# voxel-tracer/cuda-raytracing-optimized

Measured on AMD Instinct MI355X. Metric: Msamples/s (pixels x spp / s), random-spheres 1200x800x100spp, higher is better.
Workload: dtype f32; 1 GPU; random-spheres (488 spheres, LCG seed 0) 1200x800 100spp maxDepth 50, gradient sky, reference RNG stream, fp parity; spp=100, max_depth=50, spheres=488, partition=single GPU, fp_mode=parity, rng=reference, kernel_variant=0

## Files before the change

### cuda-raytracing-optimized_amd/csrc/rt_kernels_spheres.hip

```cpp
#include "rt_device.h"
#include "rt_params.h"

#include <float.h>
#include <cstdio>
#include <cstdlib>
#include <algorithm>
#include <utility>

using namespace rtd;

#if defined(RT_MODE_PARITY)
#define RT_LAUNCH_NAME rt_launch_spheres_parity
#elif defined(RT_MODE_FAST)
#define RT_LAUNCH_NAME rt_launch_spheres_fast
#else
#error "define RT_MODE_PARITY or RT_MODE_FAST"
#endif

namespace {

#ifndef RT_BOX_CUT
#define RT_BOX_CUT 12
#endif
constexpr int kWavesPerWg = 16;
// ... 95 lines not shown
    }
    for (int k = threadIdx.x; k < 3 * P.n_groups + rt_cell_f4(P.n_groups); k += (int)blockDim.x) s_grp[k] = P.groups[k];
    for (int k = threadIdx.x; k < P.n; k += (int)blockDim.x) s_sof[k] = P.slot_of[k];
    float* s_fb = reinterpret_cast<float*>(s_sof + ((P.n + 3) & ~3));
    *after = s_fb;
    unsigned char* scratch = reinterpret_cast<unsigned char*>(s_fb + (WITH_FB ? kThreads * 3 : 0));
    __syncthreads();
    return { s_sph, s_grp, s_mat, s_typ, s_org, s_sof, s_rad, scratch };
}

struct Lane {
    uint32_t rng;
    f3 col;
    f3 org, dir, atten;
    int bounce;
    bool inside;
    int s;
    int i, j;
    uint32_t pixelId;
};

struct SampleParams { rt_camera cam; int32_t nx, ny, rng_mode; };
template <bool COUNTER = true, typename PP>
__device__ __forceinline__ void start_sample(const PP& P, Lane& L) {
    if (COUNTER && P.rng_mode == RT_RNG_COUNTER) L.rng = sample_seed(L.pixelId, (uint32_t)L.s);
    const float u = ((float)L.i + rnd(L.rng)) / (float)P.nx;
    const float v = ((float)L.j + rnd(L.rng)) / (float)P.ny;
    f3 d;
    get_ray(P.cam, u, v, L.rng, L.org, d);
    L.dir = unit(d);
    L.atten = F3(1.0f, 1.0f, 1.0f);
    L.bounce = 0;
    L.inside = false;
}

__device__ __forceinline__ void init_pixel(const RtSphereParams& P, Lane& L, int i, int j, int first_sample = 0) {
    L.i = i; L.j = j;
    L.pixelId = (uint32_t)(j * P.nx + i);
    L.rng = pixel_seed(L.pixelId);
    L.col = F3(0, 0, 0);
    L.s = first_sample;
}

__device__ __forceinline__ void start_pixel(const RtSphereParams& P, Lane& L, int i, int j, int first_sample = 0) {
    init_pixel(P, L, i, j, first_sample);
    start_sample(P, L);
}

__device__ __forceinline__ void scan_group_broadcast(const RtSphereParams& P, const SceneLds& S, int g, f3 org, f3 dn, float a, Hit& h) {
    const int base = g << kSphereGroupShift;
    const float4* sp = S.sph + sidx(base);
    uint32_t mask = 0;
#pragma unroll
    for (int kk = 0; kk < kSphereGroup; kk++) {
        const float4 sph = sp[kk];
        const float ocx = org.x - sph.x;
        const float ocy = org.y - sph.y;
        const float ocz = org.z - sph.z;
        const float b = ocx * dn.x + ocy * dn.y + ocz * dn.z;
        const float c = (ocx * ocx + ocy * ocy + ocz * ocz) - sph.w;
        const float nd = a * c - b * b;
        mask = __builtin_amdgcn_alignbit(mask, __float_as_uint(nd), 31);
    }
    mask <<= (32 - kSphereGroup);
    while (mask) {
        const int lz = __clz((int)mask);
// ... 511 lines not shown
        if (reach) {
            const int at = np + (int)__builtin_amdgcn_mbcnt_hi((uint32_t)(rm >> 32), __builtin_amdgcn_mbcnt_lo((uint32_t)rm, 0u));
            w_pair[at] = (unsigned short)((r << 12) | g);
        }
        np += (int)__popcll(rm);
    }
    __builtin_amdgcn_fence(__ATOMIC_ACQ_REL, "wavefront");
    __builtin_amdgcn_wave_barrier();
    lap(12);
    for (int base = 0; base < (np << kSphereGroupShift); base += 64) {
        const int w = base + lane;
        if (w < (np << kSphereGroupShift)) {
            const unsigned pr = w_pair[w >> kSphereGroupShift];
            const int r = (int)(pr >> 12), g = (int)(pr & 0xFFFu);
            const float4 ro = w_ray[r], rd = w_ray[64 + r];
            sparse_test_slot(P, S, (g << kSphereGroupShift) + (w & (kSphereGroup - 1)), F3(ro.x, ro.y, ro.z), F3(rd.x, rd.y, rd.z), ro.w, &w_best[r]);
        }
    }
    __builtin_amdgcn_fence(__ATOMIC_ACQ_REL, "wavefront");
    __builtin_amdgcn_wave_barrier();
    Hit out = { FLT_MAX, -1, 0x7fffffff };
    if (mine) {
        const unsigned long long key = w_best[my_r];
        if (key != ~0ull) {
            out.closest = __uint_as_float((uint32_t)(key >> 32));
            out.orig = (int)(uint32_t)key;
            out.sid = S.slot_of[out.orig];
        }
    }
    lap(13);
    return out;
}

__device__ __forceinline__ Hit scan_single(const RtSphereParams& P, const SceneLds& S, int q, f3 org, f3 dn, float a) {
    const int lane = threadIdx.x & 63;
    auto bc = [&](float v) { return __int_as_float(__builtin_amdgcn_readlane(__float_as_int(v), q)); };
    const f3 O = F3(bc(org.x), bc(org.y), bc(org.z)), D = F3(bc(dn.x), bc(dn.y), bc(dn.z));
    const float A = bc(a);
    const float Ak = A - 3.814697265625e-6f;
    const int rounds = P.n_padded >> 6;
    uint32_t mask = 0;
#pragma unroll 4
    for (int r = 0; r < rounds; r++) {
        const float4 sph = S.sph[sidx((r << 6) + lane)];
        const f3 oc = O - F3(sph.x, sph.y, sph.z);
        const float b = __builtin_fmaf(oc.z, D.z, __builtin_fmaf(oc.y, D.y, oc.x * D.x));
        const float c = __builtin_fmaf(oc.z, oc.z, __builtin_fmaf(oc.y, oc.y, __builtin_fmaf(oc.x, oc.x, -sph.w)));
        const float v = __builtin_fmaf(Ak, c, -__builtin_fmaf(b, b, 7.62939453125e-6f * sph.w));
        mask |= (__float_as_uint(v) >> 31) << r;
    }
    Hit h = { FLT_MAX, -1, 0x7fffffff };
    while (mask) {
        const int r = __builtin_ctz(mask);
        mask &= mask - 1u;
        const int k = (r << 6) + lane;
        const float t = sphere_hit_exact(S.sph[sidx(k)], O, D, A, P.t_min, FLT_MAX);
        const int o = S.orig[k];
        if (o != 0x7fffffff && t < FLT_MAX) accept(h, t, k, o);
    }
    unsigned long long found = __ballot(h.closest < FLT_MAX);
    uint32_t st = __float_as_uint(FLT_MAX);
    int sk = -1, so = 0x7fffffff;
    while (found) {
        const int bq = __builtin_ctzll(found);
        found &= found - 1;
        const uint32_t tb = (uint32_t)__builtin_amdgcn_readlane(__float_as_int(h.closest), bq);
        const int ob = __builtin_amdgcn_readlane(h.orig, bq);
        if (tb < st || (tb == st && ob < so)) { st = tb; so = ob; sk = __builtin_amdgcn_readlane(h.sid, bq); }
    }
// ... 330 lines not shown
            const uint32_t rank = s_base[cls] + atomicAdd(&s_cnt[cls], 1u);
            const uint32_t at = s_start[cls] + (uint32_t)(((unsigned long long)rank * s_stride[cls]) % s_n[cls]);
            const size_t px = (size_t)(packed >> 16) * P.nx + (packed & 0xFFFFu);
            if (P.ord_rec) {
                P.ord_rec[2 * (size_t)at] = P.px_state[px];
                P.ord_rec[2 * (size_t)at + 1] = make_float4(__uint_as_float(packed), __uint_as_float(P.px_rays[px]), 0.0f, 0.0f);
            } else {
                P.order[at] = packed;
                P.ord_state[at] = P.px_state[px];
                P.ord_rays[at] = P.px_rays[px];
            }
        }
    }
}


struct BitField {
    int shift, mask;
    constexpr int put(int value) const { return value << shift; }
};
constexpr int kCfgCull = 1 << 0;
constexpr int kCfgChainSingle = 1 << 1;
constexpr int kCfgSingleRay = 1 << 2;
constexpr BitField kCfgPool = { 3, 0x1F };
constexpr BitField kCfgBoost = { 8, 0xFF };
constexpr BitField kCfgSparseMax = { 16, 0xFF };
constexpr int kCfgDbgLight = 1 << 29;
constexpr int kCfgP1Segments = 1 << 30;
constexpr BitField kChainEvery = { 0, 0xFF };
constexpr BitField kChainWaves = { 8, 0xF };
constexpr BitField kChainPixels = { 12, 0xF };
constexpr BitField kChainHeavyThr = { 16, 0xFF };
constexpr BitField kChainLists = { 24, 0xF };
constexpr BitField caps_list(int c) { return { 4 * c, 0xF }; }
constexpr BitField kCapsMidWaves = { 16, 0xF };
constexpr BitField kCapsMidCap = { 20, 0xFF };

template <int PHASE, int CLS, bool CHUNKED, bool DBG, int SCENE = 0, int LEAN = 0>
__global__ void __launch_bounds__(kThreads, (LEAN & 4) ? 6 : 4) k_render_spheres_queue(const RtSphereParams P, uint32_t stride, int cfg, int chain_cfg, int caps) {
    extern __shared__ __align__(16) unsigned char smem[];
    float* unused;
    const SceneLds S = stage_scene<false, SCENE>(P, smem, &unused);

    const bool cull = (cfg & kCfgCull) != 0;
    const int boost = (cfg >> kCfgBoost.shift) & kCfgBoost.mask;
    const int sparse_max = (cfg >> kCfgSparseMax.shift) & kCfgSparseMax.mask;
    const int tiles_x = (P.nx + 7) >> 3;
    const int tiles_y = (P.part.local_rows + 7) >> 3;
    const uint32_t padded = (uint32_t)tiles_x * (uint32_t)tiles_y * 64u;
    constexpr int n_cls = CLS == 2 ? kCostClasses : (CLS == 1 ? 3 : 0);
    __shared__ uint32_t s_cls_base[kCostClasses], s_cls_pos[kCostClasses + 1], s_cls_stride[kCostClasses];
    __shared__ uint32_t s_q[8 * kXcdQueues];
    const uint32_t xq = (CLS == 2 && P.xcd_queues == kXcdQueues) ? (uint32_t)kXcdQueues : 1u;
    const uint32_t myx = xq > 1u ? ((uint32_t)__builtin_amdgcn_s_getreg((31 << 11) | 20) & (uint32_t)(kXcdQueues - 1)) : 0u;
    if (threadIdx.x < xq) {
        const uint32_t x = threadIdx.x;
        const uint32_t* const Q = P.queue + (size_t)x * kXcdQueueWords;
        const uint32_t seg = CLS == 2 ? Q[3] : 0u;
        const int n_chain = CLS == 2 ? ((chain_cfg >> kChainLists.shift) & kChainLists.mask) : 0;
        const int n_heavy_end = CLS == 2 ? kChainClasses + kHeavyClasses : 1;
        uint32_t pos = 0, nA = 0, n0 = 0;
        for (int c = 0; c < n_cls; c++) {
            const uint32_t n = Q[4 + c];
            if (x == myx) {
                s_cls_base[c] = CLS == 2 ? seg + pos : (uint32_t)c * padded;
                s_cls_pos[c] = pos;
                s_cls_stride[c] = (CLS != 1 || c == n_cls - 1) ? 1u : coprime_stride_of(n);
            }
            if (c < n_chain) nA += n; else if (c < n_heavy_end) n0 += n;
// ... 2 lines not shown
        if (x == myx) for (int c = n_cls; c <= kCostClasses; c++) s_cls_pos[c] = pos;
        const uint32_t total_px = n_cls ? pos - nA : padded;
        const uint32_t n_rest = total_px - n0;
        const uint32_t wgs = xq > 1u ? max(gridDim.x / xq, 1u) : gridDim.x;
        uint32_t spread = wgs * blockDim.x;
        if (nA > 0u) spread -= min(spread - 64u, ((wgs + (uint32_t)(chain_cfg & kChainEvery.mask) - 1u) / (uint32_t)(chain_cfg & kChainEvery.mask)) * (uint32_t)((chain_cfg >> kChainWaves.shift) & kChainWaves.mask) * 64u);
        uint32_t* const sq = s_q + 8 * x;
        sq[0] = nA; sq[1] = n0; sq[2] = total_px * (CHUNKED ? (uint32_t)P.chunks : 1u); sq[3] = spread;
        sq[4] = (n0 > 0u && n0 <= spread && (spread - n0) <= n_rest) ? 1u : 0u;
        sq[5] = 0u;
        if (CLS == 2 && ((caps >> kCapsMidWaves.shift) & kCapsMidWaves.mask) != 0 && n0 > 0u) { sq[5] = 1u; sq[2] = n_rest; sq[4] = 0u; }
        sq[6] = seg;
    }
    __syncthreads();
    int role = 2;
    if (CLS == 2 && s_q[8 * myx] > 0u && (int)(threadIdx.x >> 6) < ((chain_cfg >> kChainWaves.shift) & kChainWaves.mask) && (blockIdx.x % (uint32_t)(chain_cfg & kChainEvery.mask)) == 0u) role = 0;
    else if (CLS == 2 && s_q[8 * myx + 5] != 0u && (int)(threadIdx.x >> 6) < ((chain_cfg >> kChainWaves.shift) & kChainWaves.mask) + ((caps >> kCapsMidWaves.shift) & kCapsMidWaves.mask)) role = 1;
    const int mid_cap = (caps >> kCapsMidCap.shift) & kCapsMidCap.mask;
    uint32_t stolen = 0;
    int ccls = 7;

    Lane L;
    L.col = F3(0, 0, 0);
    L.org = F3(0, 0, 0); L.dir = F3(0, 0, 1);
    int lr = 0;
    int chunk = 0, s_end_lane = 0;
    auto s_end_of = [&]() -> int { return CHUNKED ? s_end_lane : (PHASE == 1 ? P.s_split : (PHASE == 2 ? P.ns : min(P.ns, P.spw))); };
    uint32_t nrays = 0, groups_done = 0, boxes_done = 0;
    bool have_pixel = false;
    uint32_t pix_rays = 0;
    bool exhausted = false;
    uint32_t pool_next = 0, pool_end = 0;
    float* fbf = reinterpret_cast<float*>(P.fb);
    auto sample_params = [&]() {
        typedef const __attribute__((address_space(4))) float* ColdF;
        typedef const __attribute__((address_space(4))) int32_t* ColdI;
        unsigned long long base = (unsigned long long)P.self;
        asm volatile("" : "+s"(base));
        SampleParams sp;
        ColdF cf = (ColdF)(base + offsetof(RtSphereParams, cam));
        float* dst = reinterpret_cast<float*>(&sp.cam);
#pragma unroll
        for (int k = 0; k < (int)(sizeof(rt_camera) / 4); k++) dst[k] = cf[k];
        sp.nx = *(ColdI)(base + offsetof(RtSphereParams, nx)); sp.ny = *(ColdI)(base + offsetof(RtSphereParams, ny));
        sp.rng_mode = *(ColdI)(base + offsetof(RtSphereParams, rng_mode));
        return sp;
    };
    unsigned long long* const wdbg = DBG ? P.wave_dbg : nullptr;
    const unsigned long long dbg_t0 = wdbg ? __builtin_amdgcn_s_memrealtime() : 0ull;
    const unsigned long long dbg_t0c = wdbg ? __builtin_amdgcn_s_memtime() : 0ull;
    unsigned long long dbg_tex = 0ull;
    uint32_t dbg_iters = 0, dbg_coop_iters = 0, dbg_coop_rays = 0, dbg_maxpix = 0;
    unsigned long long dbg_tm[16] = { 0, 0, 0, 0, 0, 0, 0, 0, 0, 0, 0, 0, 0, 0, 0, 0 };
    float dbg_grab = 0.0f, dbg_p1 = 0.0f;

    bool need_sample = false;
    auto finish = [&](bool fin, bool now, f3 sample) {
        if (fin) {
            if (DBG && P.counters && (isnan(sample.x) || isnan(sample.y) || isnan(sample.z))) ray_stat<DBG>(P, RT_STAT_NAN);
            L.col = L.col + sample;
            L.s++;
            if (L.s < s_end_of()) {
                if (now) start_sample<PHASE == 0>(sample_params(), L); else need_sample = true;
            } else {
                if (PHASE == 1) {
                    const size_t px = (size_t)lr * P.nx + L.i;
                    P.px_state[px] = make_float4(L.col.x, L.col.y, L.col.z, __uint_as_float(L.rng));
                    P.px_rays[px] = pix_rays;
                } else if (!CHUNKED) {
                    const f3 out = L.col / (float)P.ns;
                    *reinterpret_cast<float3*>(fbf + ((size_t)(P.fb_global_rows ? L.j : lr) * P.nx + L.i) * 3) = make_float3(out.x, out.y, out.z);
                    float4* const acc = rt_cold_arg<float4*>(offsetof(RtSphereParams, acc_state));
                    if (acc) {
                        const size_t px = (size_t)lr * P.nx + L.i;
                        acc[px] = make_float4(L.col.x, L.col.y, L.col.z, __uint_as_float(L.rng));
                        rt_cold_arg<uint32_t*>(offsetof(RtSphereParams, acc_rays))[px] = pix_rays;
                    }
                } else {
                    float* dst = reinterpret_cast<float*>(P.partial) + (((size_t)lr * P.nx + L.i) * (uint32_t)P.chunks + (uint32_t)chunk) * 3;
                    dst[0] = L.col.x; dst[1] = L.col.y; dst[2] = L.col.z;
                }
                if (wdbg) {
                    dbg_maxpix = max(dbg_maxpix, pix_rays);
                    if (PHASE == 2)
                        P.px_state[(size_t)lr * P.nx + L.i] = make_float4(dbg_grab, (float)(__builtin_amdgcn_s_memrealtime() - dbg_t0) * 1e-5f, (float)pix_rays, dbg_p1);
                }
                have_pixel = false;
            }
        }
    };

    uint32_t poison_at = (PHASE == 1 && P.poison_fb) ? 2u + 2u * ((blockIdx.x * (blockDim.x >> 6) + (threadIdx.x >> 6)) % 24u) : ~0u;
    uint32_t iter_no = 0;
    while (true) {
        if (PHASE == 1 && iter_no++ == poison_at) poison_rows(P, (size_t)blockIdx.x * blockDim.x + threadIdx.x, (size_t)gridDim.x * blockDim.x);
        const bool dbg_timers = DBG && wdbg && (cfg & kCfgDbgLight) == 0;
        const unsigned long long t_refill = dbg_timers ? __builtin_amdgcn_s_memtime() : 0ull;
        while (!exhausted) {
            const unsigned long long live_m = __ballot(have_pixel);
            int cap = 64;
            if (CLS == 2 && (role == 1 || __ballot(have_pixel && ccls == 6) != 0ull)) cap = mid_cap;
            if (CLS == 2 && (role == 0 || __ballot(have_pixel && ccls < 6) != 0ull)) {
                cap = (chain_cfg >> kChainPixels.shift) & kChainPixels.mask;
                if (__ballot(have_pixel && ccls == 2) != 0ull) cap = min(cap, (caps >> caps_list(2).shift) & caps_list(2).mask);
                if (__ballot(have_pixel && ccls == 1) != 0ull) cap = min(cap, (caps >> caps_list(1).shift) & caps_list(1).mask);
                if (__ballot(have_pixel && ccls == 0) != 0ull) cap = min(cap, caps & caps_list(0).mask);
            }
            const int allowed = cap - (int)__popcll(live_m);
            if (allowed <= 0) break;
            const unsigned long long idle_m = ~live_m;
            const uint32_t idle_rank = __builtin_amdgcn_mbcnt_hi((uint32_t)(idle_m >> 32), __builtin_amdgcn_mbcnt_lo((uint32_t)idle_m, 0u));
            const unsigned long long need = __ballot(!have_pixel && idle_rank < (uint32_t)allowed);
            if (need == 0ull) break;
            const uint32_t cnt = (role == 0 && (cfg & kCfgChainSingle)) ? 1u : (uint32_t)__popcll(need);
            const uint32_t qx = xq > 1u ? ((myx + (stolen >> 1)) & (uint32_t)(kXcdQueues - 1)) : 0u;
            const uint32_t* const sq = s_q + 8 * qx;
            const uint32_t total = sq[2];
            if (pool_next >= pool_end) {
                const bool leftovers = (stolen & 1u) != 0u;
                const uint32_t grab = leftovers ? 1u : ((CHUNKED || PHASE == 1) ? max(cnt, 128u) : ((PHASE == 2 && role == 2) ? max(cnt, (uint32_t)((cfg >> kCfgPool.shift) & kCfgPool.mask) * 4u) : cnt));
                const uint32_t limit = (role == 0 || leftovers) ? sq[0] : (role == 1 ? sq[1] : total);
                uint32_t b = 0;
                if ((threadIdx.x & 63) == 0) b = atomicAdd(P.queue + (size_t)qx * kXcdQueueWords + ((role == 0 || leftovers) ? 1 : (role == 1 ? 2 : 0)), grab);
// ... 125 lines not shown
                const uint32_t heavy_thr = (uint32_t)((chain_cfg >> kChainHeavyThr.shift) & kChainHeavyThr.mask);
                const bool heavy = have_pixel && pix_rays > heavy_thr * (uint32_t)(L.s - chunk * P.spw + 2);
                const unsigned long long hm = __ballot(heavy);
                if (hm == 0ull) break;
                const int h = (int)__popcll(hm);
                const int hr = (int)__builtin_amdgcn_mbcnt_hi((uint32_t)(hm >> 32), __builtin_amdgcn_mbcnt_lo((uint32_t)hm, 0u));
                const int start = h > kSparseRays ? ((x - 1) * kSparseRays) % h : 0;
                int d = hr - start;
                if (d < 0) d += h;
                sel = heavy && d < kSparseRays;
            }
            if (sel) { nrays++; pix_rays++; }
            if (x > 0 || steps == 1) __builtin_amdgcn_s_setprio(3); else __builtin_amdgcn_s_setprio(0);
            f3 sample;
            const bool done = trace_rays<false, DBG, (LEAN & 1) != 0, (LEAN & 2) ? ((LEAN & 32) ? 4 : ((LEAN & 16) ? 2 : 1)) : 0, (LEAN & 8) != 0>(P, S, L, sel, -1, cull, groups_done, boxes_done, sample, sparse_max, dbg_timers ? dbg_tm : nullptr, (cfg & kCfgSingleRay) != 0);
            if (dbg_timers) { dbg_tm[x > 0 ? 9 : 8] += 1ull; }
            finish(done && sel, steps > 1, sample);
        }
    }

    if (PHASE == 1 && poison_at != ~0u && iter_no <= poison_at) poison_rows(P, (size_t)blockIdx.x * blockDim.x + threadIdx.x, (size_t)gridDim.x * blockDim.x);
    if (DBG && P.counters) {
        atomicAdd(&P.counters->rays, (unsigned long long)nrays);
        atomicAdd(&P.counters->prim_tests, (unsigned long long)nrays * (unsigned long long)P.n);
        atomicAdd(&P.counters->exec_tests, (unsigned long long)groups_done * 4ull);
        atomicAdd(&P.counters->box_tests, (unsigned long long)boxes_done);
    }
    if (wdbg) atomicMax(wdbg + 65536ull * 8 - 1, (unsigned long long)dbg_maxpix);
    if (wdbg && (threadIdx.x & 63) == 0) {
        unsigned long long* w = wdbg + ((size_t)blockIdx.x * (blockDim.x >> 6) + (threadIdx.x >> 6)) * 8;
        w[0] = dbg_t0; w[1] = dbg_tex; w[2] = __builtin_amdgcn_s_memrealtime();
        w[3] = dbg_iters; w[4] = dbg_coop_iters; w[5] = dbg_coop_rays;
        w[6] = ((unsigned long long)__builtin_amdgcn_s_getreg((31 << 11) | 20) << 32) | (unsigned)__builtin_amdgcn_s_getreg((31 << 11) | 4);
        w[7] = 1;
        for (int k = 0; k < 8; k++) atomicAdd(wdbg + 65534ull * 8 + k, dbg_tm[k]);
        if (dbg_coop_iters >= 2000ull) {
            for (int k = 0; k < 8; k++) atomicAdd(wdbg + 65532ull * 8 + k, dbg_tm[k]);
            for (int k = 0; k < 4; k++) atomicAdd(wdbg + 65531ull * 8 + k, dbg_tm[10 + k]);
            atomicAdd(wdbg + 65531ull * 8 + 4, dbg_coop_iters); atomicAdd(wdbg + 65531ull * 8 + 5, 1ull);
            atomicAdd(wdbg + 65531ull * 8 + 6, __builtin_amdgcn_s_memtime() - dbg_t0c);
        }
        atomicAdd(wdbg + 65533ull * 8 + 0, dbg_tm[8]); atomicAdd(wdbg + 65533ull * 8 + 1, dbg_tm[9]);
    }
}

}

namespace {
__global__ void __launch_bounds__(256) k_sum_chunks(const RtSphereParams P) {
    const size_t px = (size_t)blockIdx.x * 256 + threadIdx.x;
    if (px >= (size_t)P.part.local_rows * P.nx) return;
    const float* src = reinterpret_cast<const float*>(P.partial) + px * P.chunks * 3;
    f3 col = F3(src[0], src[1], src[2]);
    for (int c = 1; c < P.chunks; c++) col = col + F3(src[3 * c], src[3 * c + 1], src[3 * c + 2]);
    const f3 out = col / (float)P.ns;
    float* dst = reinterpret_cast<float*>(P.fb) + px * 3;
    dst[0] = out.x; dst[1] = out.y; dst[2] = out.z;
}
}

constexpr size_t kStaticLds = 1024;
constexpr size_t kLdsPerCu = 160 * 1024 - kStaticLds;
static size_t lds_bytes(int n_padded, int n, bool with_fb, int scene = 0, int waves = kWavesPerWg, bool onepass = false) {
    const size_t test_data = (size_t)(n_padded + n_padded / kSphereGroup) * 16 + (size_t)(n_padded / kSphereGroup) * 48 + (size_t)rt_cell_f4(n_padded / kSphereGroup) * 16;
    const size_t scratch = (size_t)waves * ws_total(onepass);
    if (scene == 1) return scratch;
    if (scene == 2) return test_data + (size_t)n_padded * 4 + scratch;
// ... 31 lines not shown
    const int scene = scene_form(p, false);
    const auto kern = scene == 0 ? k_guides_spheres<0> : (scene == 1 ? k_guides_spheres<1> : k_guides_spheres<2>);
    const unsigned long long total = (unsigned long long)((p.nx + 7) / 8) * ((p.part.local_rows + 7) / 8) * 64ull;
    const dim3 grid((unsigned)((total + kThreads - 1) / kThreads));
    return launch_with_lds(kern, grid, dim3(kThreads), lds_bytes(p.n_padded, p.n, false, scene, 0), stream, p, g);
}
#endif

constexpr int kLeanBasic = 1 << 0, kLeanOneList = 1 << 1, kLeanSixWaves = 1 << 2, kLeanAxes3 = 1 << 3, kLeanWords2 = 1 << 4, kLeanWords4 = 1 << 5;
using KindsFull = std::integer_sequence<int, 1, 3, 7, 11, 15, 19, 27, 35, 43>;
using KindsChunked = std::integer_sequence<int, 1, 3, 7>;
using KindsHybrid = std::integer_sequence<int, 1, 35, 43>;
using KindsStamped = std::integer_sequence<int, 3>;

template <int... LEANS>
constexpr bool in_kinds(std::integer_sequence<int, LEANS...>, int lean) { return ((lean == LEANS) || ...); }
constexpr bool built(int scene, bool chunked, int lean) {
    if (lean == 0) return true;
    if (scene == 0) return chunked ? in_kinds(KindsChunked{}, lean) : in_kinds(KindsFull{}, lean);
    return scene == 2 && !chunked && in_kinds(KindsHybrid{}, lean);
}
constexpr int clip_lean(int scene, bool chunked, int lean) {
    return built(scene, chunked, lean) ? lean : (built(scene, chunked, lean & kLeanBasic) ? (lean & kLeanBasic) : 0);
}

enum class SphereFrame {
    Tiles,
    GlobalSingle,
    TwoDispatch,
    TwoDispatchResume,
    ClassifiedSingle,
    PlainSingle,
};
enum class SpherePlanError { None, Mid, Tune };
constexpr int kFirstSamples = 2;

struct SpherePlan {
    SpherePlanError error = SpherePlanError::None;
    SphereFrame frame = SphereFrame::PlainSingle;
    bool legacy = false;
    int coop_below = -1;
    int cull = 1;
    int scene = 0;
    bool chunked = false;
    int lean = 0;
    int lean_dbg = 0;
    int threads = kThreads;
    size_t lds = 0;
    unsigned blocks = 1, blocks_y = 1;
    unsigned cls_blocks = 1;
    uint32_t stride = 1;
    uint32_t stride1 = 1;
    int cfg = 0, cfg1 = 0, chain_cfg = 0, caps = 0;
    bool sum_chunks = false;
};

enum { kTuneChainEvery, kTuneChainWaves, kTuneHeavyThr, kTuneChainLists, kTuneBoost, kTuneChainPixels, kTuneList0, kTuneList1, kTuneList2, kTuneFields };
constexpr int kCapsNoTiers = caps_list(0).put(4) | caps_list(1).put(4) | caps_list(2).put(4) | caps_list(3).put(4);

static SpherePlan plan_spheres(const RtSphereParams& p, int variant, const RtSwitches& sw, int cus) {
    SpherePlan pl;
    const int cb_bits = (variant >> 16) & 0xFF;
    pl.legacy = cb_bits != 0 && cb_bits != 255;
    pl.cull = ((variant >> 26) & 1) ? 0 : 1;
    const size_t tile_lds = lds_bytes(p.n_padded, p.n, true, 0, kWavesPerWg);
    if (((variant & 0xFF) == 1 || pl.legacy) && !p.global_scene && tile_lds <= kLdsPerCu) {
        pl.frame = SphereFrame::Tiles;
// ... 35 lines not shown
    if ((lean & (kLeanOneList | kLeanWords2 | kLeanWords4)) == kLeanOneList && sw.lean6_pixels > 0 && (long long)p.nx * p.part.local_rows >= sw.lean6_pixels &&
        2 * (lds_bytes(p.n_padded, p.n, false, 0, 12, true) + kStaticLds) <= (size_t)160 * 1024) { lean |= kLeanSixWaves; waves = 12; default_wgs = 2; }
    pl.lean = lean;
    pl.threads = 64 * waves;
    pl.lds = lds_bytes(p.n_padded, p.n, false, pl.scene, waves, (lean & kLeanOneList) != 0);
    int wg_per_cu = (variant >> 8) & 0xFF;
    if (wg_per_cu == 0) wg_per_cu = default_wgs;
    const long long total_px = (long long)((p.nx + 7) / 8) * ((p.part.local_rows + 7) / 8) * 64;
    const long long useful = (total_px + pl.threads - 1) / pl.threads;
    pl.blocks = (unsigned)std::max(1ll, std::min((long long)cus * wg_per_cu, useful));
    pl.cls_blocks = (unsigned)((total_px + kThreads - 1) / kThreads);
    if (order_mode == 0 && ((pl.scene == 2 && !sw.hybrid_two) || pl.scene == 1)) order_mode = 2;
    if (order_mode != 1 && total_px > 64) pl.stride = rt_coprime_stride((unsigned long long)total_px);
    const bool resume = p.acc_first > 0 && p.acc_state && p.acc_rays;
    if (pl.scene == 1) pl.frame = SphereFrame::GlobalSingle;
    else if (two_dispatch(order_mode, p.ns >= 8 || resume)) pl.frame = resume ? SphereFrame::TwoDispatchResume : SphereFrame::TwoDispatch;
    else if ((order_mode == 0 || order_mode == 3) && p.order != nullptr) pl.frame = SphereFrame::ClassifiedSingle;
    else pl.frame = SphereFrame::PlainSingle;
    pl.sum_chunks = pl.chunked;

    if (sw.mid_waves < 0 || sw.mid_waves > 12 || sw.mid_cap < 1 || sw.mid_cap > 64) { pl.error = SpherePlanError::Mid; return pl; }
    const int pb = (variant >> 27) & 7;
    int sparse_max = 4 + 4 * ((variant >> 30) & 3);
    if (cb_bits == 255) sparse_max = 0;
    const int boost = (pb == 7 || cb_bits == 255) ? 0 : (pb == 0 ? 1 : pb);
    int t[kTuneFields] = { 1, waves == 16 ? 3 : (waves >= 10 ? 2 : 1), 8, kChainClasses, boost, kSparseRays, 1, 4, 4 };
    if (sw.tune) {
        t[kTuneChainWaves] = waves == 16 ? 3 : 1;
        for (int i = 0; i < sw.tune->n; i++) t[i] = sw.tune->v[i];
        const int lo[kTuneFields] = { 1, 0, 1, 0, 0, 1, 1, 1, 1 }, hi[kTuneFields] = { 255, waves, 255, 15, 255, 15, 15, 15, 15 };
        for (int i = 0; i < kTuneFields; i++)
            if (t[i] < lo[i] || t[i] > hi[i]) { pl.error = SpherePlanError::Tune; return pl; }
    }
    pl.chain_cfg = kChainEvery.put(t[kTuneChainEvery]) | kChainWaves.put(t[kTuneChainWaves]) | kChainPixels.put(t[kTuneChainPixels]) | kChainHeavyThr.put(t[kTuneHeavyThr]) |
                   kChainLists.put(t[kTuneChainLists]);
    pl.caps = caps_list(0).put(t[kTuneList0]) | caps_list(1).put(t[kTuneList1]) | caps_list(2).put(t[kTuneList2]) | caps_list(3).put(t[kTuneChainPixels]) |
              kCapsMidWaves.put(sw.mid_waves) | kCapsMidCap.put(sw.mid_cap);
    pl.cfg = (pl.cull ? kCfgCull : 0) | (sw.chain_single ? kCfgChainSingle : 0) | (sw.single_ray ? kCfgSingleRay : 0) | kCfgPool.put((sw.pool / 4) & kCfgPool.mask) |
             kCfgBoost.put(t[kTuneBoost]) | kCfgSparseMax.put(sparse_max) | (sw.wave_debug_light ? kCfgDbgLight : 0);
    pl.stride1 = p.p1_tile_major == 1 ? 1u : pl.stride;
    pl.cfg1 = pl.cfg;
    if (p.p1_tile_major == 2 && total_px > 512) {
        pl.stride1 = rt_coprime_stride((unsigned long long)total_px >> 3);
        pl.cfg1 |= kCfgP1Segments;
    }
    return pl;
}

template <int PHASE, int CLS, bool CHUNKED, bool DBG, int SCENE, int LEAN = 0> struct SphereQueueForm {};

template <int PHASE, int CLS, bool CHUNKED, bool DBG, int SCENE, int LEAN>
static hipError_t launch_sphere_queue(SphereQueueForm<PHASE, CLS, CHUNKED, DBG, SCENE, LEAN>, const RtSphereParams& q, const SpherePlan& pl, hipStream_t stream,
                                      uint32_t stride, int cfg, int caps) {
    const hipError_t e = launch_with_lds(k_render_spheres_queue<PHASE, CLS, CHUNKED, DBG, SCENE, LEAN>, dim3(pl.blocks), dim3(pl.threads), pl.lds, stream, q, stride, cfg, pl.chain_cfg, caps);
    rt_note_launch(RT_KERNEL_SPHERE_QUEUE, PHASE, CLS, CHUNKED, DBG, SCENE, LEAN, pl.threads, pl.blocks);
    return e;
}

template <int PHASE, int CLS, bool CHUNKED, bool DBG, int SCENE, int... LEANS, typename Go>
static bool launch_kind_of(std::integer_sequence<int, LEANS...>, int lean, Go&& go, hipError_t& e) {
    return ((lean == LEANS && ((e = go(SphereQueueForm<PHASE, CLS, CHUNKED, DBG, SCENE, LEANS>{})), true)) || ...);
}

template <int PHASE, int CLS, bool CHUNKED>
static hipError_t launch_queue_form(const SpherePlan& pl, const RtSphereParams& q, hipStream_t stream, uint32_t stride, int cfg, int caps = kCapsNoTiers) {
    const bool counting = q.wave_dbg != nullptr || q.counters != nullptr;
    auto go = [&](auto form) -> hipError_t { return launch_sphere_queue(form, q, pl, stream, stride, cfg, caps); };
    hipError_t e = hipErrorInvalidValue;
// ... 2 lines not shown
        return e;
    }
    if (counting && q.counters == nullptr && pl.scene == 0 && !CHUNKED && PHASE != 0 && launch_kind_of<PHASE, CLS, false, true, 0>(KindsStamped{}, pl.lean_dbg, go, e)) return e;
    if (counting) return pl.scene == 2 ? go(SphereQueueForm<PHASE, CLS, CHUNKED, true, 2>{}) : go(SphereQueueForm<PHASE, CLS, CHUNKED, true, 0>{});
    if (pl.lean == 0) return pl.scene == 2 ? go(SphereQueueForm<PHASE, CLS, CHUNKED, false, 2>{}) : go(SphereQueueForm<PHASE, CLS, CHUNKED, false, 0>{});
    if (pl.scene == 0 && !CHUNKED) launch_kind_of<PHASE, CLS, false, false, 0>(KindsFull{}, pl.lean, go, e);
    if (pl.scene == 0 && CHUNKED) launch_kind_of<PHASE, CLS, true, false, 0>(KindsChunked{}, pl.lean, go, e);
    if (pl.scene == 2 && !CHUNKED) launch_kind_of<PHASE, CLS, false, false, 2>(KindsHybrid{}, pl.lean, go, e);
    return e;
}

hipError_t RT_LAUNCH_NAME(const RtSphereParams& p, int variant, const RtSwitches& sw, hipStream_t stream) {
    if (!p.self) return hipErrorInvalidValue;
    int dev = 0, cus = 256;
    if (hipGetDevice(&dev) == hipSuccess) (void)hipDeviceGetAttribute(&cus, hipDeviceAttributeMultiprocessorCount, dev);
    const SpherePlan pl = plan_spheres(p, variant, sw, cus);
    auto wait_fb = [&]() -> hipError_t {
        if (!p.poison_fb) return hipSuccess;
        hipLaunchKernelGGL(k_poison_fb, dim3(512), dim3(256), 0, stream, p);
        return hipGetLastError();
    };
    hipError_t e;
    if (pl.frame == SphereFrame::Tiles) {
        if ((e = wait_fb()) != hipSuccess) return e;
        e = launch_with_lds(pl.legacy ? k_render_spheres_tiles<true> : k_render_spheres_tiles<false>, dim3(pl.blocks, pl.blocks_y), dim3(kThreads), pl.lds, stream, p, pl.coop_below, pl.cull);
        rt_note_launch(RT_KERNEL_SPHERE_TILES, 0, pl.legacy ? 1 : 0, 0, 0, 0, 0, kThreads, pl.blocks * pl.blocks_y);
        return e;
    }
    if (!p.queue) return hipErrorInvalidValue;
    if ((e = hipMemsetAsync(p.queue, 0, 256, stream)) != hipSuccess) return e;
    if (pl.error == SpherePlanError::Tune)
        fprintf(stderr, "rt error: RT_TUNE=%s out of range (chain_every 1..255, chain_waves 0..%d, heavy_thr 1..255, n_chain 0..15, boost 0..255, "
                        "chain_pixels 1..15, chain_pixels of list 0 / 1 / 2 1..15)\n", sw.tune->text.c_str(), kWavesPerWg);
    if (pl.error != SpherePlanError::None) return hipErrorInvalidValue;
    if (pl.frame == SphereFrame::TwoDispatch || pl.frame == SphereFrame::TwoDispatchResume) {
        RtSphereParams q = p;
        if (pl.frame == SphereFrame::TwoDispatchResume) {
            q.px_state = p.acc_state; q.px_rays = p.acc_rays; q.s_split = p.acc_first;
            e = wait_fb();
        } else {
            q.phase = 1; q.s_split = kFirstSamples;
            e = launch_queue_form<1, 0, false>(pl, q, stream, pl.stride1, pl.cfg1);
        }
        if (e != hipSuccess) return e;
        if ((e = hipMemsetAsync(p.queue, 0, sizeof(uint32_t) * kXcdQueues * kXcdQueueWords, stream)) != hipSuccess) return e;
        if ((e = order_pixels_by_cost(q, stream)) != hipSuccess) return e;
        q.phase = 2;
        if (sw.wave_debug_phase) q.wave_dbg = nullptr;
        return launch_queue_form<2, 2, false>(pl, q, stream, pl.stride, pl.cfg, pl.caps);
    }
    const bool classified = pl.frame == SphereFrame::ClassifiedSingle;
    if (classified) {
        e = launch_with_lds(pl.scene == 2 ? k_classify_spheres<2> : k_classify_spheres<0>, dim3(pl.cls_blocks), dim3(kThreads), pl.lds, stream, p);
        if (e != hipSuccess) return e;
    }
    if ((e = wait_fb()) != hipSuccess) return e;
    if (classified) e = pl.chunked ? launch_queue_form<0, 1, true>(pl, p, stream, pl.stride, pl.cfg) : launch_queue_form<0, 1, false>(pl, p, stream, pl.stride, pl.cfg);
    else e = pl.chunked ? launch_queue_form<0, 0, true>(pl, p, stream, pl.stride, pl.cfg) : launch_queue_form<0, 0, false>(pl, p, stream, pl.stride, pl.cfg);
    if (e != hipSuccess) return e;
    if (pl.sum_chunks) {
        const size_t npx = (size_t)p.part.local_rows * p.nx;
        hipLaunchKernelGGL(k_sum_chunks, dim3((unsigned)((npx + 255) / 256)), dim3(256), 0, stream, p);
    }
    return hipGetLastError();
}
```

### cuda-raytracing-optimized_amd/csrc/rt_params.h

```cpp
#pragma once

#include <hip/hip_runtime.h>
#include <stdint.h>

#include <optional>
#include <string>

#include "../../include/rt_types.h"
#include "../../include/rt_api.h"

constexpr int kSphereGroupShift = 4;
constexpr int kSphereGroup = 1 << kSphereGroupShift;
constexpr int kCellCount = 64;
constexpr int kCellWordsMax = 8;
__host__ __device__ inline int rt_cell_words(int n_groups) { const int w = (n_groups + 31) / 32; return w <= kCellWordsMax ? w : 0; }
__host__ __device__ inline int rt_cell_f4(int n_groups) { return (6 * kCellCount * rt_cell_words(n_groups)) / 4; }

struct RtPartition {
    int32_t stripe_rows;
    int32_t rank;
    int32_t world;
    int32_t local_rows;
};

// ... 114 lines not shown
    int32_t p1_segments;
    float4* acc_state;
    int32_t acc_first;
};

template <typename T>
__device__ __forceinline__ T rt_cold_arg(size_t offset) {
    unsigned long long base = (unsigned long long)__builtin_amdgcn_kernarg_segment_ptr();
    asm volatile("" : "+s"(base));
    return *reinterpret_cast<const __attribute__((address_space(4))) T*>(base + offset);
}

size_t rt_sphere_kernel_lds_bytes(int n_padded, int n);
hipError_t rt_order_pixels_by_cost(const RtSphereParams& q, hipStream_t stream);

struct RtTune {
    std::string text;
    int n = 0;
    int v[9] = {};
};

struct RtSwitches {
    bool xcd_queues = true;
    bool ord_packed = true;
    int p1_tile = 2;
    std::optional<std::string> wave_debug;
    bool fb_direct = false;
    bool fb_poison = true;
    bool box_cells = true;
    bool compact_leaves = true;
    bool ext_fb_no_register = false;
    bool cleanup_device_reset = false;
    int top_thr = 384;
    bool basic = true;
    bool onepass = true;
    long long lean6_pixels = 2600000;
    bool hybrid_two = false;
    int mid_waves = 0, mid_cap = 16;
    bool chain_single = true;
    bool single_ray = true;
    int pool = 4;
    bool wave_debug_light = false;
    bool wave_debug_phase = false;
    std::optional<RtTune> tune;
    bool mesh_lean = true;
    bool mesh_tile_order = false;
    bool mesh_two = true;
    int mesh_split = 2;
    int mesh_heavy = 5;
    int mesh_rounds = 2;
    bool mesh_rev = false;
    int mesh_chain_thr = 448;
    int mesh_chain_lanes = 6;
    int mesh_chain_frac = 8;
    std::optional<std::string> mesh_diag_file;
};
RtSwitches rt_read_switches();

inline uint32_t rt_coprime_stride(unsigned long long n) {
    auto gcd = [](unsigned long long a, unsigned long long b) { while (b) { const unsigned long long t = a % b; a = b; b = t; } return a; };
    unsigned long long cand = (unsigned long long)((double)n * 0.6180339887) | 1ull;
    while (gcd(cand, n) != 1ull) cand += 2;
    return (uint32_t)(cand % n);
}

hipError_t rt_launch_spheres_parity(const RtSphereParams& p, int variant, const RtSwitches& sw, hipStream_t stream);
// ... 15 lines not shown
```

### cuda-raytracing-optimized_amd/csrc/rt_renderer.hip

```cpp
#include <hip/hip_runtime.h>

#include <algorithm>
#include <chrono>
#include <climits>
#include <cmath>
#include <cstdio>
#include <cstdlib>
#include <cstring>
#include <functional>
#include <string>
#include <vector>

#include "../../include/rt_api.h"
#include "rt_params.h"
#include "rt_denoise.h"
#include "rt_accumulate.h"

namespace {

#define HIP_CHECK(expr) hip_check((expr), #expr, __FILE__, __LINE__)

void hip_check(hipError_t result, const char* func, const char* file, int line) {
    if (result != hipSuccess) {
        fprintf(stderr, "HIP error = %s at %s:%d '%s' \n", hipGetErrorString(result), file, line, func);
// ... 917 lines not shown
    const char* v = getenv(name);
    return v && v[0] == '1';
}

int env_int(const char* name, int dflt) {
    const char* v = getenv(name);
    return v ? atoi(v) : dflt;
}

std::optional<std::string> env_str(const char* name) {
    const char* v = getenv(name);
    if (!v) return std::nullopt;
    return std::string(v);
}

}

RtSwitches rt_read_switches() {
    RtSwitches s;
    s.xcd_queues = env_flag("RT_XCD_QUEUES", s.xcd_queues);
    s.ord_packed = env_flag("RT_ORD_PACKED", s.ord_packed);
    const int p1_tile = env_int("RT_P1_TILE", s.p1_tile);
    s.p1_tile = (p1_tile >= 0 && p1_tile <= 2) ? p1_tile : 0;
    s.wave_debug = env_str("RT_WAVE_DEBUG");

    s.fb_direct = env_flag("RT_FB_DIRECT", s.fb_direct);
    s.fb_poison = env_flag("RT_FB_POISON", s.fb_poison);
    s.box_cells = env_flag("RT_BOX_CELLS", s.box_cells);
    s.compact_leaves = env_flag("RT_COMPACT_LEAVES", s.compact_leaves);
    s.ext_fb_no_register = env_one("RT_EXT_FB_NO_REGISTER");
    s.cleanup_device_reset = env_one("RT_CLEANUP_DEVICE_RESET");

    const int top_thr = env_int("RT_TOP_THR", s.top_thr);
    if (top_thr >= 320) s.top_thr = top_thr;
    s.basic = env_flag("RT_BASIC", s.basic);
    s.onepass = env_flag("RT_ONEPASS", s.onepass);
    if (const auto v = env_str("RT_LEAN6_PIXELS")) s.lean6_pixels = atoll(v->c_str());
    s.hybrid_two = env_one("RT_HYBRID_TWO");
    if (const auto v = env_str("RT_MID")) sscanf(v->c_str(), "%d,%d", &s.mid_waves, &s.mid_cap);
    s.chain_single = env_flag("RT_CHAIN_SINGLE", s.chain_single);
    s.single_ray = env_flag("RT_SINGLE_RAY", s.single_ray);
    s.pool = env_int("RT_POOL", s.pool);
    s.wave_debug_light = env_one("RT_WAVE_DEBUG_LIGHT");
    s.wave_debug_phase = env_one("RT_WAVE_DEBUG_PHASE");
    if (const auto v = env_str("RT_TUNE")) {
        RtTune& t = s.tune.emplace();
        t.text = *v;
        t.n = std::max(0, sscanf(v->c_str(), "%d,%d,%d,%d,%d,%d,%d,%d,%d", &t.v[0], &t.v[1], &t.v[2], &t.v[3], &t.v[4], &t.v[5], &t.v[6], &t.v[7], &t.v[8]));
    }

    s.mesh_lean = env_flag("RT_MESH_LEAN", s.mesh_lean);
    const auto order = env_str("RT_MESH_ORDER");
    s.mesh_tile_order = order && (*order)[0] == 't';
    s.mesh_two = env_flag("RT_MESH_TWO", s.mesh_two);
    s.mesh_split = std::max(1, env_int("RT_MESH_SPLIT", s.mesh_split));
    s.mesh_heavy = env_int("RT_MESH_HEAVY", s.mesh_heavy);
    s.mesh_rounds = env_int("RT_MESH_ROUNDS", s.mesh_rounds);
    s.mesh_rev = env_one("RT_MESH_REV");
    s.mesh_chain_thr = std::max(17, env_int("RT_MESH_CHAIN_THR", s.mesh_chain_thr));
    s.mesh_chain_lanes = std::min(64, std::max(0, env_int("RT_MESH_CHAIN_LANES", s.mesh_chain_lanes)));
    s.mesh_chain_frac = env_int("RT_MESH_CHAIN_FRAC", s.mesh_chain_frac) & 0xF;
    s.mesh_diag_file = env_str("RT_MESH_DIAG_FILE");
    return s;
}

extern "C" {

// ... 187 lines not shown
```

Before: 8446 Msamples/s.

## Serve chain-class pixels in a noinline wave-uniform chain loop

Adds a noinline chain_loop function that chain-role waves in phase 2 run first. Each wave grabs whole heavy pixels from the per-XCD queue with CAS and traces them with a wave-uniform scan_single, which skips the readlane broadcasts. The loop reloads the parameter block from the kernarg pointer so the main kernel's register pressure does not carry into this hot path. The waves also raise their priority with s_setprio. The default chain_loop=4 enables it, which risks load imbalance and extra call overhead, and the RT_TOP_THR minimum is relaxed.

```diff
diff --git a/cuda-raytracing-optimized_amd/csrc/rt_kernels_spheres.hip b/cuda-raytracing-optimized_amd/csrc/rt_kernels_spheres.hip
--- a/cuda-raytracing-optimized_amd/csrc/rt_kernels_spheres.hip
+++ b/cuda-raytracing-optimized_amd/csrc/rt_kernels_spheres.hip
@@ -151,6 +151,20 @@
     L.atten = F3(1.0f, 1.0f, 1.0f);
     L.bounce = 0;
     L.inside = false;
+}
+
+__device__ __forceinline__ SampleParams cold_sample_params(unsigned long long base) {
+    typedef const __attribute__((address_space(4))) float* ColdF;
+    typedef const __attribute__((address_space(4))) int32_t* ColdI;
+    asm volatile("" : "+s"(base));
+    SampleParams sp;
+    ColdF cf = (ColdF)(base + offsetof(RtSphereParams, cam));
+    float* dst = reinterpret_cast<float*>(&sp.cam);
+#pragma unroll
+    for (int k = 0; k < (int)(sizeof(rt_camera) / 4); k++) dst[k] = cf[k];
+    sp.nx = *(ColdI)(base + offsetof(RtSphereParams, nx)); sp.ny = *(ColdI)(base + offsetof(RtSphereParams, ny));
+    sp.rng_mode = *(ColdI)(base + offsetof(RtSphereParams, rng_mode));
+    return sp;
 }
 
 __device__ __forceinline__ void init_pixel(const RtSphereParams& P, Lane& L, int i, int j, int first_sample = 0) {
@@ -728,9 +742,10 @@
     return out;
 }
 
+template <bool UNIFORM = false>
 __device__ __forceinline__ Hit scan_single(const RtSphereParams& P, const SceneLds& S, int q, f3 org, f3 dn, float a) {
     const int lane = threadIdx.x & 63;
-    auto bc = [&](float v) { return __int_as_float(__builtin_amdgcn_readlane(__float_as_int(v), q)); };
+    auto bc = [&](float v) { return UNIFORM ? v : __int_as_float(__builtin_amdgcn_readlane(__float_as_int(v), q)); };
     const f3 O = F3(bc(org.x), bc(org.y), bc(org.z)), D = F3(bc(dn.x), bc(dn.y), bc(dn.z));
     const float A = bc(a);
     const float Ak = A - 3.814697265625e-6f;
@@ -1127,9 +1142,100 @@
 constexpr BitField kChainPixels = { 12, 0xF };
 constexpr BitField kChainHeavyThr = { 16, 0xFF };
 constexpr BitField kChainLists = { 24, 0xF };
+constexpr BitField kChainLoop = { 28, 0x7 };
 constexpr BitField caps_list(int c) { return { 4 * c, 0xF }; }
 constexpr BitField kCapsMidWaves = { 16, 0xF };
 constexpr BitField kCapsMidCap = { 20, 0xFF };
+
+struct ChainLoopStats { uint32_t pixels, rays, maxpix; };
+template <bool DBG>
+__device__ __attribute__((noinline)) ChainLoopStats chain_loop(unsigned long long queue_check, SceneLds S, uint32_t x, uint32_t loop_end, uint32_t first_pos, unsigned long long dbg_t0) {
+    RtSphereParams P;
+    static_assert(sizeof(RtSphereParams) % 4 == 0, "chain_loop copies the parameter block by words");
+    auto uni = [](uint32_t v) { return (uint32_t)__builtin_amdgcn_readfirstlane(v); };
+    queue_check = ((unsigned long long)uni((uint32_t)(queue_check >> 32)) << 32) | uni((uint32_t)queue_check);
+    constexpr unsigned long long kExplicitArgs = (sizeof(RtSphereParams) + sizeof(uint32_t) + 3 * sizeof(int) + 7ull) & ~7ull;
+    const unsigned long long kernarg = (unsigned long long)__builtin_amdgcn_implicitarg_ptr() - kExplicitArgs;
+    x = uni(x); loop_end = uni(loop_end); first_pos = uni(first_pos);
+    dbg_t0 = ((unsigned long long)uni((uint32_t)(dbg_t0 >> 32)) << 32) | uni((uint32_t)dbg_t0);
+    const __attribute__((address_space(4))) uint32_t* const arg_words = (const __attribute__((address_space(4))) uint32_t*)kernarg;
+#pragma unroll
+    for (int k = 0; k < (int)(sizeof(RtSphereParams) / 4); k++) reinterpret_cast<uint32_t*>(&P)[k] = arg_words[k];
+    ChainLoopStats stats = { 0u, 0u, 0u };
+    if ((unsigned long long)P.queue != queue_check) return stats;
+    const bool stamps = DBG && P.wave_dbg != nullptr;
+    float* const fbf = reinterpret_cast<float*>(P.fb);
+    uint32_t* const ctr = P.queue + (size_t)x * kXcdQueueWords + 1;
+    while (true) {
+        uint32_t pos = ~0u;
+        if ((threadIdx.x & 63) == 0) {
+            uint32_t cur = __hip_atomic_load(ctr, __ATOMIC_RELAXED, __HIP_MEMORY_SCOPE_AGENT);
+            while (cur < loop_end) {
+                const uint32_t seen = atomicCAS(ctr, cur, cur + 1u);
+                if (seen == cur) { pos = cur; break; }
+                cur = seen;
+            }
+        }
+        pos = __builtin_amdgcn_readfirstlane(pos);
+        if (pos == ~0u) break;
+        const uint32_t opos = first_pos + pos;
+        float4 st4;
+        uint32_t p, c_rays;
+        if (P.ord_rec) {
+            st4 = P.ord_rec[2 * (size_t)opos];
+            const float4 rec1 = P.ord_rec[2 * (size_t)opos + 1];
+            p = __float_as_uint(rec1.x);
+            c_rays = __float_as_uint(rec1.y);
+        } else {
+            p = P.order[opos];
+            st4 = P.ord_state[opos];
+            c_rays = P.ord_rays[opos];
+        }
+        const int ci = (int)(p & 0xFFFFu), clr = (int)(p >> 16);
+        if (!(ci < P.nx && clr < P.part.local_rows)) continue;
+        Lane C;
+        C.i = ci; C.j = global_row(P.part, clr);
+        C.pixelId = (uint32_t)(C.j * P.nx + ci);
+        C.rng = __float_as_uint(st4.w);
+        C.col = F3(st4.x, st4.y, st4.z);
+        C.s = P.s_split;
+        auto vary = [](auto& v) { asm volatile("" : "+v"(v)); };
+        vary(C.rng);
+        const float c_grab = stamps ? (float)(__builtin_amdgcn_s_memrealtime() - dbg_t0) * 1e-5f : 0.0f;
+        const uint32_t c_p1 = c_rays;
+        int fresh = 1;
+        while (true) {
+            vary(fresh); vary(C.s);
+            if (fresh) { start_sample<false>(cold_sample_params((unsigned long long)P.self), C); fresh = 0; }
+            int inside = C.inside ? 1 : 0;
+            vary(C.bounce); vary(inside);
+            C.inside = inside != 0;
+            c_rays++;
+            const f3 dn = unit(C.dir);
+            const float a = dot(dn, dn);
+            const Hit h = scan_single<true>(P, S, 0, C.org, dn, a);
+            f3 sample;
+            if (shade<false, true>(P, S, C, dn, h, sample)) {
+                C.col = C.col + sample;
+                C.s++;
+                if (C.s >= P.ns) break;
+                fresh = 1;
+            }
+        }
+        if ((threadIdx.x & 63) == 0) {
+            const f3 out = C.col / (float)P.ns;
+            *reinterpret_cast<float3*>(fbf + ((size_t)(P.fb_global_rows ? C.j : clr) * P.nx + ci) * 3) = make_float3(out.x, out.y, out.z);
+            if (P.acc_state) {
+                const size_t px = (size_t)clr * P.nx + ci;
+                P.acc_state[px] = make_float4(C.col.x, C.col.y, C.col.z, __uint_as_float(C.rng));
+                P.acc_rays[px] = c_rays;
+            }
+            if (stamps) P.px_state[(size_t)clr * P.nx + ci] = make_float4(c_grab, (float)(__builtin_amdgcn_s_memrealtime() - dbg_t0) * 1e-5f, (float)c_rays, (float)c_p1);
+        }
+        if (stamps) { stats.maxpix = max(stats.maxpix, c_rays); stats.pixels++; stats.rays += c_rays - c_p1; }
+    }
+    return stats;
+}
 
 template <int PHASE, int CLS, bool CHUNKED, bool DBG, int SCENE = 0, int LEAN = 0>
 __global__ void __launch_bounds__(kThreads, (LEAN & 4) ? 6 : 4) k_render_spheres_queue(const RtSphereParams P, uint32_t stride, int cfg, int chain_cfg, int caps) {
@@ -1198,20 +1304,7 @@
     bool exhausted = false;
     uint32_t pool_next = 0, pool_end = 0;
     float* fbf = reinterpret_cast<float*>(P.fb);
-    auto sample_params = [&]() {
-        typedef const __attribute__((address_space(4))) float* ColdF;
-        typedef const __attribute__((address_space(4))) int32_t* ColdI;
-        unsigned long long base = (unsigned long long)P.self;
-        asm volatile("" : "+s"(base));
-        SampleParams sp;
-        ColdF cf = (ColdF)(base + offsetof(RtSphereParams, cam));
-        float* dst = reinterpret_cast<float*>(&sp.cam);
-#pragma unroll
-        for (int k = 0; k < (int)(sizeof(rt_camera) / 4); k++) dst[k] = cf[k];
-        sp.nx = *(ColdI)(base + offsetof(RtSphereParams, nx)); sp.ny = *(ColdI)(base + offsetof(RtSphereParams, ny));
-        sp.rng_mode = *(ColdI)(base + offsetof(RtSphereParams, rng_mode));
-        return sp;
-    };
+    auto sample_params = [&]() { return cold_sample_params((unsigned long long)P.self); };
     unsigned long long* const wdbg = DBG ? P.wave_dbg : nullptr;
     const unsigned long long dbg_t0 = wdbg ? __builtin_amdgcn_s_memrealtime() : 0ull;
     const unsigned long long dbg_t0c = wdbg ? __builtin_amdgcn_s_memtime() : 0ull;
@@ -1255,6 +1348,18 @@
             }
         }
     };
+
+    uint32_t dbg_loop_px = 0, dbg_loop_rays = 0;
+    if constexpr (PHASE == 2 && CLS == 2 && !CHUNKED && SCENE == 0 && (LEAN & 1) != 0) {
+        const int n_chain = (chain_cfg >> kChainLists.shift) & kChainLists.mask;
+        const int loop_lists = min((chain_cfg >> kChainLoop.shift) & kChainLoop.mask, min(n_chain, kChainClasses));
+        if (role == 0 && loop_lists > 0 && P.n_padded <= 2048) {
+            __builtin_amdgcn_s_setprio(3);
+            const ChainLoopStats st = chain_loop<DBG>((unsigned long long)P.queue, S, myx, __builtin_amdgcn_readfirstlane(s_cls_pos[loop_lists]), __builtin_amdgcn_readfirstlane(s_q[8 * myx + 6]), dbg_t0);
+            if (wdbg) { dbg_maxpix = max(dbg_maxpix, st.maxpix); dbg_loop_px = st.pixels; dbg_loop_rays = st.rays; }
+            if (loop_lists >= n_chain) role = 2;
+        }
+    }
 
     uint32_t poison_at = (PHASE == 1 && P.poison_fb) ? 2u + 2u * ((blockIdx.x * (blockDim.x >> 6) + (threadIdx.x >> 6)) % 24u) : ~0u;
     uint32_t iter_no = 0;
@@ -1446,7 +1551,7 @@
         w[0] = dbg_t0; w[1] = dbg_tex; w[2] = __builtin_amdgcn_s_memrealtime();
         w[3] = dbg_iters; w[4] = dbg_coop_iters; w[5] = dbg_coop_rays;
         w[6] = ((unsigned long long)__builtin_amdgcn_s_getreg((31 << 11) | 20) << 32) | (unsigned)__builtin_amdgcn_s_getreg((31 << 11) | 4);
-        w[7] = 1;
+        w[7] = 1ull | ((unsigned long long)(dbg_loop_px & 0xFFFFFFu) << 8) | ((unsigned long long)dbg_loop_rays << 32);
         for (int k = 0; k < 8; k++) atomicAdd(wdbg + 65534ull * 8 + k, dbg_tm[k]);
         if (dbg_coop_iters >= 2000ull) {
             for (int k = 0; k < 8; k++) atomicAdd(wdbg + 65532ull * 8 + k, dbg_tm[k]);
@@ -1544,7 +1649,7 @@
     ClassifiedSingle,
     PlainSingle,
 };
-enum class SpherePlanError { None, Mid, Tune };
+enum class SpherePlanError { None, Mid, Tune, ChainLoop };
 constexpr int kFirstSamples = 2;
 
 struct SpherePlan {
@@ -1646,8 +1751,9 @@
         for (int i = 0; i < kTuneFields; i++)
             if (t[i] < lo[i] || t[i] > hi[i]) { pl.error = SpherePlanError::Tune; return pl; }
     }
+    if (sw.chain_loop < 0 || sw.chain_loop > kChainClasses) { pl.error = SpherePlanError::ChainLoop; return pl; }
     pl.chain_cfg = kChainEvery.put(t[kTuneChainEvery]) | kChainWaves.put(t[kTuneChainWaves]) | kChainPixels.put(t[kTuneChainPixels]) | kChainHeavyThr.put(t[kTuneHeavyThr]) |
-                   kChainLists.put(t[kTuneChainLists]);
+                   kChainLists.put(t[kTuneChainLists]) | kChainLoop.put(sw.chain_loop);
     pl.caps = caps_list(0).put(t[kTuneList0]) | caps_list(1).put(t[kTuneList1]) | caps_list(2).put(t[kTuneList2]) | caps_list(3).put(t[kTuneChainPixels]) |
               kCapsMidWaves.put(sw.mid_waves) | kCapsMidCap.put(sw.mid_cap);
     pl.cfg = (pl.cull ? kCfgCull : 0) | (sw.chain_single ? kCfgChainSingle : 0) | (sw.single_ray ? kCfgSingleRay : 0) | kCfgPool.put((sw.pool / 4) & kCfgPool.mask) |
@@ -1716,6 +1822,7 @@
     if (pl.error == SpherePlanError::Tune)
         fprintf(stderr, "rt error: RT_TUNE=%s out of range (chain_every 1..255, chain_waves 0..%d, heavy_thr 1..255, n_chain 0..15, boost 0..255, "
                         "chain_pixels 1..15, chain_pixels of list 0 / 1 / 2 1..15)\n", sw.tune->text.c_str(), kWavesPerWg);
+    if (pl.error == SpherePlanError::ChainLoop) fprintf(stderr, "rt error: RT_CHAIN_LOOP=%d out of range (chain lists served by the chain loop: 0..%d)\n", sw.chain_loop, kChainClasses);
     if (pl.error != SpherePlanError::None) return hipErrorInvalidValue;
     if (pl.frame == SphereFrame::TwoDispatch || pl.frame == SphereFrame::TwoDispatchResume) {
         RtSphereParams q = p;
diff --git a/cuda-raytracing-optimized_amd/csrc/rt_params.h b/cuda-raytracing-optimized_amd/csrc/rt_params.h
--- a/cuda-raytracing-optimized_amd/csrc/rt_params.h
+++ b/cuda-raytracing-optimized_amd/csrc/rt_params.h
@@ -170,6 +170,7 @@
     bool ext_fb_no_register = false;
     bool cleanup_device_reset = false;
     int top_thr = 384;
+    int chain_loop = 4;
     bool basic = true;
     bool onepass = true;
     long long lean6_pixels = 2600000;
diff --git a/cuda-raytracing-optimized_amd/csrc/rt_renderer.hip b/cuda-raytracing-optimized_amd/csrc/rt_renderer.hip
--- a/cuda-raytracing-optimized_amd/csrc/rt_renderer.hip
+++ b/cuda-raytracing-optimized_amd/csrc/rt_renderer.hip
@@ -973,7 +973,8 @@
     s.cleanup_device_reset = env_one("RT_CLEANUP_DEVICE_RESET");
 
     const int top_thr = env_int("RT_TOP_THR", s.top_thr);
-    if (top_thr >= 320) s.top_thr = top_thr;
+    if (top_thr >= 17) s.top_thr = top_thr;
+    s.chain_loop = env_int("RT_CHAIN_LOOP", s.chain_loop);
     s.basic = env_flag("RT_BASIC", s.basic);
     s.onepass = env_flag("RT_ONEPASS", s.onepass);
     if (const auto v = env_str("RT_LEAN6_PIXELS")) s.lean6_pixels = atoll(v->c_str());
```

New measurement: 7410 Msamples/s. -12.3%, worse.
